# holicc/qurious

Measured on AMD Instinct MI355X. Metric: rows/s on TPC-H Q1 scan+agg and Q3 hash-join, SF10, 1/2/4/8 MI355X, higher is better.
Workload: dtype i128

## Files before the change

### qurious_amd/csrc/agg.cpp

```cpp
#include <hip/hip_runtime_api.h>

#include <algorithm>
#include <cfloat>
#include <cmath>
#include <chrono>
#include <cstdio>
#include <cstdlib>
#include <map>

#include "codegen.hpp"
#include "common.hpp"
#include "device/qhip_status.h"
#include "hostcol.hpp"
#include "jit.hpp"
#include "kargs_host.hpp"
#include "kernels.hpp"
#include "relops.hpp"

namespace qhip {
static uint64_t g_learn_tick = 0;


void HostColumn::init_fixed(const DType& t, int64_t n) {
  type = t; length = n; null_count = 0;
// ... 652 lines not shown
        items_dev.alloc(item_first.size() * 4);
        QHIP_HIP_CHECK(hipMemcpyAsync(items_dev.ptr, item_first.data(), item_first.size() * 4, hipMemcpyHostToDevice, s));
        HReduceLaunch rl;
        rl.records = records.as<uint64_t>();
        rl.item_first = items_dev.as<uint32_t>();
        rl.n_items = n_items;
        HAggLaunch Lp = L;
        Lp.l_nslots = l_nslots_p;
        void* rargs[] = {&rl, &Lp};
        if (wide) {
          std::shared_ptr<Module> m_wide = get_module(ctx, plan.source, "qk_agg_reduce_wide");
          const unsigned rgrid = (unsigned)std::min<uint64_t>(n_items, (uint64_t)ctx->num_cus * 2);
          QHIP_HIP_CHECK(hipModuleLaunchKernel(m_wide->fn, rgrid, 1, 1, 1024, 1, 1, (unsigned)((size_t)l_nslots_p * slot_bytes), s, rargs, nullptr));
        } else {
          const unsigned rgrid = (unsigned)std::min<uint64_t>(n_items, (uint64_t)ctx->num_cus * 4);
          QHIP_HIP_CHECK(hipModuleLaunchKernel(m_red->fn, rgrid, 1, 1, 256, 1, 1, (unsigned)((size_t)l_nslots_p * slot_bytes), s, rargs, nullptr));
        }
        QHIP_HIP_CHECK(sync_stream(s));
      }
      }

    } else if (N > 0 && parts) {
      dense.alloc((size_t)guess * slot_bytes + 8);
      dense_dev = dense.as<uint64_t>();
      L.part_runs = parts->runs; L.part_stride = parts->stride;
      L.dense_out = dense_dev + 1; L.dense_counter = status_dev + 16; L.dense_cap = guess;
      L.n_parts = (uint32_t)parts->n_parts;
      L.part_max = (uint32_t)std::max<int64_t>(1024, env_int("QHIP_AGG_PARTS_MAX_FACTOR", 4) * ((N + parts->n_parts - 1) / parts->n_parts));
      const unsigned pgrid = grid + (unsigned)((uint64_t)N / L.part_max) + 1;
      std::shared_ptr<Module> pmod = get_module(ctx, plan.source, "qk_filter_agg_parts");
      QHIP_HIP_CHECK(hipModuleLaunchKernel(pmod->fn, pgrid, 1, 1, 1024, 1, 1, (unsigned)lds_bytes, ctx->stream, args, nullptr));
    } else if (N > 0) {
      if (wide) {
        std::shared_ptr<Module> wmod = get_module(ctx, plan.source, "qk_filter_agg_wide");
        QHIP_HIP_CHECK(hipModuleLaunchKernel(wmod->fn, grid, 1, 1, 1024, 1, 1, (unsigned)lds_bytes, ctx->stream, args, nullptr));
      } else if (cons) {
        std::shared_ptr<Module> cmod = get_module(ctx, plan.source, "qk_filter_agg_cons");
        QHIP_HIP_CHECK(hipModuleLaunchKernel(cmod->fn, grid, 1, 1, 256, 1, 1, (unsigned)lds_bytes, ctx->stream, args, nullptr));
      } else {
        QHIP_HIP_CHECK(hipModuleLaunchKernel(mod->fn, grid, 1, 1, 256, 1, 1, (unsigned)lds_bytes, ctx->stream, args, nullptr));
      }
    }
    time_mark(ctx, 1);
    uint32_t* const counter_dev = status_dev + 16;
    pre_copied = 0;
    if (plan.W == 0) {
      QHIP_HIP_CHECK(hipMemcpyAsync(status_pinned, status_dev, sizeof(status), hipMemcpyDeviceToHost, ctx->stream));
      QHIP_HIP_CHECK(hipMemcpyAsync(pre_host, table_dev, (size_t)slot_bytes, hipMemcpyDeviceToHost, ctx->stream));
    } else {
      if (use_arena) {
        dense_dev = (uint64_t*)(arena->as<uint8_t>() + zero_bytes) ;
        pre_copied = std::min(PRE, guess);
        const bool direct = env_int("QHIP_AGG_PINNED_SLOTS", 1) != 0;
        launch_compact_slots(table_dev, total_slots, plan.slot_words, dense_dev + 1, counter_dev, guess, ctx->stream, direct ? pre_host + 1 : nullptr, pre_copied);
        QHIP_HIP_CHECK(hipMemcpyAsync(status_pinned, status_dev, 64 + 8, hipMemcpyDeviceToHost, ctx->stream));
        if (!direct) QHIP_HIP_CHECK(hipMemcpyAsync(pre_host + 1, dense_dev + 1, (size_t)pre_copied * slot_bytes, hipMemcpyDeviceToHost, ctx->stream));
      } else {
        if (!parts) { dense.alloc((size_t)guess * slot_bytes + 8); dense_dev = dense.as<uint64_t>(); }
        bool utf8_key = false;
        for (auto& kd : plan.keys) utf8_key = utf8_key || kd.type.id == QHIP_UTF8;
        spec_enqueued = false;
        const bool will_spec = replicas == 1 && plan.last_groups >= dev_threshold && !utf8_key && env_int("QHIP_AGG_NO_SPECULATIVE_FINALIZE", 0) == 0;
        const bool direct = !will_spec && !parts && env_int("QHIP_AGG_PINNED_SLOTS", 1) != 0;
        launch_compact_slots(table_dev, total_slots, plan.slot_words, dense_dev + 1, counter_dev, guess, ctx->stream, direct ? pre_host + 1 : nullptr,
                             std::min(PRE, guess));
        if (will_spec) {
          spec = DevFinal();
          const int ncols = n_groups + n_aggs;
          enqueue_device_finalize(spec, dense_dev + 1, guess, counter_dev, status_dev + 32, status_pinned + 32);
          spec_enqueued = true;
          QHIP_HIP_CHECK(hipMemcpyAsync(status_pinned, status_dev, (size_t)(32 + QS_WORDS + ncols) * 4, hipMemcpyDeviceToHost, ctx->stream));
        } else {
          QHIP_HIP_CHECK(hipMemcpyAsync(status_pinned, status_dev, 64 + 8, hipMemcpyDeviceToHost, ctx->stream));
          pre_copied = std::min(PRE, guess);
          if (!direct) QHIP_HIP_CHECK(hipMemcpyAsync(pre_host + 1, dense_dev + 1, (size_t)pre_copied * slot_bytes, hipMemcpyDeviceToHost, ctx->stream));
        }
      }
    }
    if (use_arena) {
      QHIP_HIP_CHECK(hipEventRecord(ctx->ev[2], ctx->stream));
      QHIP_HIP_CHECK(hipMemsetAsync(arena->ptr, 0, zero_bytes, ctx->stream));
      plan.arena_clean = true;
      mark("launched");
      QHIP_HIP_CHECK(sync_event(ctx->ev[2]));
    } else {
      mark("launched");
      QHIP_HIP_CHECK(sync_stream(ctx->stream));
    }
    memcpy(status, status_pinned, sizeof(status));
    if (env_int("QHIP_AGG_PROF", 0)) {
      const double waves = (double)grid * (block / 64);
      fprintf(stderr, "[qhip agg prof] rows %lld grid %u x %d: loads+eval %.0f  cache %.0f  table updates %.0f  cached keys -> table %.0f  merge %.0f  (x256 cycles per wavefront)\n",
              (long long)N, grid, block, status_pinned[8] / waves, status_pinned[9] / waves, status_pinned[10] / waves, status_pinned[11] / waves, status_pinned[12] / waves);
    }
    mark("synchronised");
    trace_point("aggregate: back from its wait");
    verify_pending_sizes(ctx);
    if (in->rows_dev && in->deferred_count() == 0 && n_groups > 0) return no_batches_out();
    if (ctx->timing) QHIP_HIP_CHECK(hipEventElapsedTime(&main_ms, ctx->ev[0], ctx->ev[1]));
    check_status_words(status);
    if (!status[QS_OVERFLOW]) break;
    if (replicas == 1 && cap >= cap_max) fail(QHIP_HIP_ERROR, "group table overflow at maximum capacity (internal error)");
    cap = replicas > 1 ? std::min<uint32_t>(cap_max, std::max<uint32_t>(cap * 16, 1u << 18)) : (uint32_t)std::min<uint64_t>((uint64_t)cap * 16, cap_max);
    replicas = 1;
    ++retries;
  }

  const uint32_t lds_used = status[QS_LDS_USED];
// ... 257 lines not shown
```

### qurious_amd/csrc/device/qhip_device.hpp

```cpp
#pragma once

typedef unsigned char u8;
typedef unsigned short u16;
typedef unsigned int u32;
typedef unsigned long long u64;
typedef long long i64;
typedef __int128 i128;
typedef unsigned __int128 u128;

#define QH_MAXC 24
#define QH_MAXL 24
#define QH_WAVE 64
#define QH_BLOCK 256

struct KCol {
  const void* v;
  const u8* n;
  const u8* d;
};

struct KArgs {
  KCol c[QH_MAXC];
  u64 lit_lo[QH_MAXL];
  i64 lit_hi[QH_MAXL];
// ... 1437 lines not shown
  qh_mask_load<P>(a, A, first, mine, 0, lane);
  qh_mask_load<P>(a, B, first, mine, 1, lane);
  asm volatile("" ::: "memory");
  __builtin_amdgcn_sched_barrier(0);
#define QH_MASK_TRIP(X3, X1, J)                                    \
  qh_mask_finish<P>(a, X3, mask, wave_count, nwords, lane, err);   \
  qh_mask_load<P>(a, X1, first, mine, (J), lane);                  \
  asm volatile("" ::: "memory");                                   \
  __builtin_amdgcn_sched_barrier(0);
  for (i64 j = 0; j < mine; j += 3) {
    QH_MASK_TRIP(A, C, j + 2)
    QH_MASK_TRIP(B, A, j + 3)
    QH_MASK_TRIP(C, B, j + 4)
  }
#undef QH_MASK_TRIP
  qh_report(status, err);
}

__device__ __forceinline__ u32 qh_region(u64 h, u32 n_regions) { return (u32)(((h >> 32) * (u64)n_regions) >> 32); }
template <int W>
__device__ __forceinline__ u32 qh_join_find(const u64* table, u32 base, u32 mask, const u64* k, u32 s) {
  for (u32 probes = 0; probes <= mask; ++probes) {
    const u32 at = base + (s & mask);
    const u64* slot = table + (size_t)at * (1 + W);
    if (slot[0] < QH_READY) return 0xFFFFFFFFu;
    bool eq = true;
#pragma unroll
    for (int w = 0; w < W; ++w) eq &= slot[1 + w] == k[w];
    if (eq) return at;
    ++s;
  }
  return 0xFFFFFFFFu;
}
struct ProbeLaunch {
  const u64* table;
  const u64* bloom;
  const u32* count;
  const u32* start;
  const u32* rows;
  u32* ent_slot;
  u32* ent_row;
  u32* tile_nent;
  u32* tile_total;
  u32* visited;
  u32* status;
  u32 nslots, bloom_mask;
  u32 n_regions;
  u32 slot_bits, bword_bits, stage_cap;
  u32 tiles_per_wave, lds_words;
  u64 dense_min;
  u32 dense_n, dense_words;
  const u32* dense_rank;
  u32 dense_last;
};

__device__ __forceinline__ u64 qh_filter_mask(u32 x) {
  const u32 lo = (1u << (x & 31u)) | (1u << ((x >> 5) & 31u)), hi = (1u << ((x >> 10) & 31u)) | (1u << ((x >> 15) & 31u));
  return ((u64)hi << 32) | lo;
}
__device__ __forceinline__ u32 qh_filter_word(u64 h, u32 word_mask) { return (u32)(h >> 32) & word_mask; }
__device__ __forceinline__ u32 qh_rfilter_word(u64 h, u32 sb, u32 wb) { return ((u32)h >> sb) & ((1u << wb) - 1u); }
__device__ __forceinline__ u64 qh_rfilter_mask(u64 h, u32 sb, u32 wb) { return qh_filter_mask((u32)(h >> (sb + wb))); }

template <class P>
struct QhProbeTile {
  typename P::Raw raw[P::PROBE_R];
  u64 k[P::PROBE_R][P::W];
  u64 fw[P::PROBE_R], fm[P::PROBE_R];
  u32 at[P::PROBE_R];
  u64 st[P::PROBE_R], kw[P::PROBE_R][P::W];
  bool ok[P::PROBE_R];
  i64 tile;
  bool live;
};
struct QhProbeCtx { bool regions; u32 smask; int lane; i64 first, mine; u32 nent, total; };

template <class P>
__device__ __forceinline__ void qh_probe_stage1(const KArgs& a, QhProbeTile<P>& x, const QhProbeCtx& c, i64 j) {
  constexpr int R = P::PROBE_R, TILE = 64 * R;
  x.live = j < c.mine;
  x.tile = x.live ? c.first + j : 0;
  const i64 tb = x.tile * TILE;
#pragma unroll
  for (int r = 0; r < R; ++r) {
    const u32 o = (u32)r * 64 + (u32)c.lane;
    P::load(a, tb, tb + (i64)o < a.nrows ? o : (u32)(a.nrows - 1 - tb), x.raw[r]);
  }
}
template <class P, bool REGIONS>
__device__ __forceinline__ void qh_probe_stage2(const KArgs& a, const ProbeLaunch& L, QhProbeTile<P>& x, const QhProbeCtx& c, u32& err) {
  constexpr int R = P::PROBE_R, TILE = 64 * R, W = P::W;
#pragma unroll
  for (int r = 0; r < R; ++r) {
    const bool inb = x.tile * TILE + r * 64 + c.lane < a.nrows;
    u32 e = 0;
    x.ok[r] = P::keys(a, x.raw[r], x.k[r], e) && inb;
    err |= (inb && x.live) ? e : 0u;
    const u64 h = qh_key_hash<W>(x.k[r]);
    const u32 reg = REGIONS ? qh_region(h, L.n_regions) : 0u;
    x.at[r] = (REGIONS ? reg << L.slot_bits : 0u) + ((u32)h & c.smask);
    x.fm[r] = REGIONS ? qh_rfilter_mask(h, L.slot_bits, L.bword_bits) : qh_filter_mask((u32)h);
    const u32 word = REGIONS ? (reg << L.bword_bits) + qh_rfilter_word(h, L.slot_bits, L.bword_bits) : qh_filter_word(h, L.bloom_mask);
    x.fw[r] = *(const u64*)((const char*)L.bloom + (size_t)((x.ok[r] ? word : 0u) << 3));
  }
}
template <class P>
// ... 8 lines not shown
      const qh_v2u64 sk = *(const qh_v2u64*)slot;
      x.st[r] = sk.x;
      x.kw[r][0] = sk.y;
    } else {
      x.st[r] = slot[0];
#pragma unroll
      for (int w = 0; w < W; ++w) x.kw[r][w] = slot[1 + w];
    }
  }
}
template <class P>
__device__ __forceinline__ void qh_probe_stage4(const ProbeLaunch& L, QhProbeTile<P>& x, QhProbeCtx& c) {
  constexpr int R = P::PROBE_R, TILE = 64 * R, W = P::W;
  const int lane = c.lane;
  u32 sid[R];
#pragma unroll
  for (int r = 0; r < R; ++r) {
    sid[r] = 0xFFFFFFFFu;
    if (x.ok[r] && x.st[r] >= QH_READY) {
      bool eq = true;
#pragma unroll
      for (int w = 0; w < W; ++w) eq &= x.kw[r][w] == x.k[r][w];
      const u32 home = x.at[r] & c.smask, base = x.at[r] & ~c.smask;
      sid[r] = eq ? x.at[r] : qh_join_find<W>(L.table, base, c.smask, x.k[r], home + 1);
      if (!L.start && sid[r] != 0xFFFFFFFFu) sid[r] = (u32)((eq ? x.st[r] : L.table[(size_t)sid[r] * (1 + W)]) - 2);
    }
  }
  if (!x.live) return;
  u32 total = 0, nent = c.nent;
#pragma unroll
  for (int r = 0; r < R; ++r) {
    const bool found = sid[r] != 0xFFFFFFFFu;
    u32 cnt = 1u;
    if (L.start) cnt = L.count[found ? sid[r] : 0u];
    total += found ? cnt : 0u;
    const u64 m = qh_ballot(found);
    if (found) {
      const size_t pos = (size_t)c.first * TILE + nent + (u32)__builtin_popcountll(m & ((1ULL << lane) - 1));
      L.ent_slot[pos] = sid[r];
      L.ent_row[pos] = (u32)(x.tile * TILE + r * 64 + lane);
    }
    nent += (u32)__builtin_popcountll(m);
  }
  c.nent = nent;
  if (L.visited) {
#pragma unroll
    for (int r = 0; r < R; ++r)
      if (sid[r] != 0xFFFFFFFFu) {
        const u32 s0 = L.start ? L.start[sid[r]] : 0u, cnt = L.start ? L.count[sid[r]] : 1u;
        for (u32 q = 0; q < cnt; ++q) { const u32 b = L.start ? L.rows[s0 + q] : sid[r]; atomicOr(&L.visited[b >> 5], 1u << (b & 31)); }
      }
  }
  c.total += (u32)qh_wave_sum_u64(total);
}

template <class P, bool REGIONS>
__device__ __forceinline__ void qh_join_probe_body(const KArgs& a, const ProbeLaunch& L) {
  constexpr int R = P::PROBE_R, TILE = 64 * R, NW = QH_BLOCK / 64;
  const i64 ntiles = (a.nrows + TILE - 1) / TILE;
  QhProbeCtx c;
  c.regions = REGIONS;
  c.smask = REGIONS ? (1u << L.slot_bits) - 1u : L.nslots - 1u;
  c.lane = qh_lane();
  const i64 wave = (i64)blockIdx.x * NW + __builtin_amdgcn_readfirstlane((int)(threadIdx.x >> 6));
  c.first = wave * (i64)L.tiles_per_wave;
  c.nent = 0; c.total = 0;
  if (c.first >= ntiles) {
    if (c.lane == 0) { L.tile_total[wave] = 0; L.tile_nent[wave] = 0; }
    return;
  }
  c.mine = ntiles - c.first < (i64)L.tiles_per_wave ? ntiles - c.first : (i64)L.tiles_per_wave;
  u32 err = 0;
  QhProbeTile<P> A, B, C;
  qh_probe_stage1<P>(a, A, c, 0);
  qh_probe_stage2<P, REGIONS>(a, L, A, c, err);
  qh_probe_stage1<P>(a, B, c, 1);
  qh_probe_stage3<P>(L, A, c);
  qh_probe_stage2<P, REGIONS>(a, L, B, c, err);
  qh_probe_stage1<P>(a, C, c, 2);
#define QH_PROBE_TRIP(X4, X3, X2, J)          \
  qh_probe_stage4<P>(L, X4, c);               \
  qh_probe_stage3<P>(L, X3, c);               \
  qh_probe_stage2<P, REGIONS>(a, L, X2, c, err);       \
  qh_probe_stage1<P>(a, X4, c, (J));
  for (i64 j = 3; j < c.mine + 3; j += 3) {
    QH_PROBE_TRIP(A, B, C, j)
    QH_PROBE_TRIP(B, C, A, j + 1)
    QH_PROBE_TRIP(C, A, B, j + 2)
  }
#undef QH_PROBE_TRIP
  if (c.lane == 0) { L.tile_total[wave] = c.total; L.tile_nent[wave] = c.nent; }
  qh_report(L.status, err);
}

struct DenseBuildLaunch {
  u32* bits;
  u32* row_of;
  u32* status;
  u64 kmin;
  u32 n;
  u32 gen;
  u8* bytes;
  u32* counters;
};
template <class P, bool DEVROWS = false>
__device__ __forceinline__ void qh_join_dense_build_body(const KArgs& a, const DenseBuildLaunch& L) {
  constexpr int R = 4;
  const i64 nrows = DEVROWS ? qh_rows(a) : a.nrows;
  const i64 tile = (i64)QH_BLOCK * R;
  u32 err = 0, dup = 0, out_of_range = 0, inserted = 0;
  const bool bytemap = L.bytes != nullptr;
  for (i64 tb = (i64)blockIdx.x * tile; tb < nrows; tb += (i64)gridDim.x * tile) {
    u64 k[R][P::W];
    bool ok[R];
#pragma unroll
    for (int r = 0; r < R; ++r) {
      const i64 i = tb + (i64)r * QH_BLOCK + threadIdx.x;
      const bool inb = i < nrows;
      u32 e = 0;
      ok[r] = P::keys(a, inb ? i : nrows - 1, k[r], e) && inb;
      err |= inb ? e : 0u;
    }
#pragma unroll
    for (int r = 0; r < R; ++r) {
      const u64 idx = k[r][0] - L.kmin;
      if (ok[r]) {
        if (idx < (u64)L.n) {
          if (bytemap) {
            L.bytes[(u32)idx] = (u8)L.gen;
            ++inserted;
          } else {
            const u32 bit = 1u << ((u32)idx & 31u);
            const u32 old = __hip_atomic_fetch_or(&L.bits[(u32)idx >> 5], bit, __ATOMIC_RELAXED, __HIP_MEMORY_SCOPE_AGENT);
            dup |= (old & bit) ? 1u : 0u;
          }
          L.row_of[(u32)idx] = (u32)(tb + (i64)r * QH_BLOCK + threadIdx.x);
        } else out_of_range = 1u;
      }
    }
  }
  qh_report(L.status, err | (out_of_range << QS_OVERFLOW));
  if (bytemap) {
    const u32 wave_rows = (u32)qh_wave_sum_u64((u64)inserted);
    if (qh_lane() == 0 && wave_rows) atomicAdd(&L.counters[0], wave_rows);
    return;
// ... 159 lines not shown
  const u64 below = (1ULL << lane) - 1;
  if (st.nbuf + (u32)TILE > st.cap) qh_dense_flush(L, st, (u64)c.first * TILE, lane);
  bool hit[R];
  u64 m[R];
#pragma unroll
  for (int r = 0; r < R; ++r) {
    const u32 word = (LDSBITS == 2 && (x.idx[r] >> 5) < L.lds_words) ? x.bl[r] : x.bw[r];
    hit[r] = x.ok[r] && ((word >> (x.idx[r] & 31u)) & 1u);
    m[r] = qh_ballot(hit[r]);
  }
  if (WIDE) {
    u32 before = 0, total = 0;
#pragma unroll
    for (int r = 0; r < R; ++r) { before += (u32)__builtin_popcountll(m[r] & below); total += (u32)__builtin_popcountll(m[r]); }
    u32 pos = st.nbuf + before;
#pragma unroll
    for (int r = 0; r < R; ++r)
      if (hit[r]) { st.idx[pos] = x.idx[r]; st.row[pos] = (u32)(x.tb + (i64)((u32)lane * R + (u32)r)); ++pos; }
    st.nbuf += total;
  } else {
    u32 n = st.nbuf;
#pragma unroll
    for (int r = 0; r < R; ++r) {
      if (hit[r]) {
        const u32 pos = n + (u32)__builtin_popcountll(m[r] & below);
        st.idx[pos] = x.idx[r];
        st.row[pos] = (u32)(x.tile * TILE + r * 64 + lane);
      }
      n += (u32)__builtin_popcountll(m[r]);
    }
    st.nbuf = n;
  }
}
template <class P, int LDSBITS, bool WIDE>
__device__ __forceinline__ void qh_join_probe_dense_body(const KArgs& a, const ProbeLaunch& L) {
  constexpr int R = P::PROBE_R, TILE = 64 * R;
  const int NW = (int)(blockDim.x >> 6);
  const u32 nbits = LDSBITS == 1 ? L.dense_words : LDSBITS == 2 ? L.lds_words : 0u;
  if (LDSBITS) {
    u32* lbits = (u32*)qh_dyn_lds;
    for (u32 w = threadIdx.x; w < nbits; w += blockDim.x) lbits[w] = ((const u32*)L.bloom)[w];
    __syncthreads();
  }
  const i64 ntiles = (a.nrows + TILE - 1) / TILE;
  QhProbeCtx c;
  c.regions = false; c.smask = 0;
  c.lane = qh_lane();
  const int wave_in_wg = __builtin_amdgcn_readfirstlane((int)(threadIdx.x >> 6));
  const i64 wave = (i64)blockIdx.x * NW + wave_in_wg;
  c.first = wave * (i64)L.tiles_per_wave;
  c.nent = 0; c.total = 0;
  if (c.first >= ntiles) {
    if (c.lane == 0) { L.tile_total[wave] = 0; L.tile_nent[wave] = 0; }
    return;
  }
  c.mine = ntiles - c.first < (i64)L.tiles_per_wave ? ntiles - c.first : (i64)L.tiles_per_wave;
  QhDenseStage st;
  st.cap = L.stage_cap;
  st.idx = (u32*)qh_dyn_lds + ((nbits + 1u) & ~1u) + (u32)wave_in_wg * 2u * L.stage_cap;
  st.row = st.idx + L.stage_cap;
  st.nbuf = 0; st.nflushed = 0;
  u32 err = 0;
  QhDenseTile<P> A, B, C;
  qh_dense_stage1<P, WIDE>(a, A, c, 0);
  qh_dense_stage1<P, WIDE>(a, B, c, 1);
  asm volatile("" ::: "memory");
  qh_dense_stage2<P, LDSBITS, WIDE>(a, L, A, c, err);
  asm volatile("" ::: "memory");
#define QH_DENSE_TRIP(X3, X2, X1, J)                   \
  qh_dense_stage3<P, LDSBITS, WIDE>(L, X3, c, st);     \
  qh_dense_stage2<P, LDSBITS, WIDE>(a, L, X2, c, err); \
  qh_dense_stage1<P, WIDE>(a, X1, c, (J));             \
  asm volatile("" ::: "memory");
  for (i64 j = 0; j < c.mine; j += 3) {
    QH_DENSE_TRIP(A, B, C, j + 2)
    QH_DENSE_TRIP(B, C, A, j + 3)
    QH_DENSE_TRIP(C, A, B, j + 4)
  }
#undef QH_DENSE_TRIP
  qh_dense_flush(L, st, (u64)c.first * TILE, c.lane);
  if (c.lane == 0) { L.tile_total[wave] = st.nflushed; L.tile_nent[wave] = st.nflushed; }
  qh_report(L.status, err);
}

struct ScatterLaunch {
  u64* entries;
  u32* first;
  u32* status;
  u32 n_regions;
  u32 rows_per_wg;
};

#define QH_SCATTER_BLOCK 1024
template <class P, bool DEVROWS = false>
__device__ __forceinline__ void qh_join_scatter_body(const KArgs& a, const ScatterLaunch& L) {
  constexpr int R = 4, W = P::W, TB = QH_SCATTER_BLOCK;
  u32* cnt = (u32*)qh_dyn_lds;
  __shared__ u32 wsum[TB / 64];
  const u32 tid = threadIdx.x, nr = L.n_regions;
  for (u32 r = tid; r <= nr; r += TB) cnt[r] = 0;
  __syncthreads();
  const i64 first = (i64)blockIdx.x * L.rows_per_wg;
  const i64 nrows = DEVROWS ? qh_rows(a) : a.nrows;
  const i64 last = first + L.rows_per_wg < nrows ? first + L.rows_per_wg : nrows;
  u32 err = 0;
  const bool single = last - first <= (i64)TB * R;
  u64 k[R][W];
  bool ok[R];
  for (int pass = 0; pass < 2; ++pass) {
    for (i64 tb = first; tb < last; tb += (i64)TB * R) {
      if (!single || pass == 0) {
#pragma unroll
        for (int r = 0; r < R; ++r) {
          const i64 i = tb + (i64)r * TB + tid;
          const bool inb = i < last;
          u32 e = 0;
          ok[r] = P::keys(a, inb ? i : last - 1, k[r], e) && inb;
          if (pass == 0) err |= inb ? e : 0u;
        }
      }
#pragma unroll
      for (int r = 0; r < R; ++r) {
        if (ok[r]) {
          const u32 reg = qh_region(qh_key_hash<W>(k[r]), nr);
          const u32 pos = atomicAdd(&cnt[reg], 1u);
          if (pass == 1) {
            u64* e = L.entries + ((size_t)first + pos) * (1 + W);
            e[0] = (u64)(tb + (i64)r * TB + tid) + 2;
#pragma unroll
            for (int w = 0; w < W; ++w) e[1 + w] = k[r][w];
          }
        }
      }
    }
    __syncthreads();
// ... 106 lines not shown
```

### qurious_amd/csrc/join.cpp

```cpp
#include <hip/hip_runtime_api.h>

#include <algorithm>
#include <map>

#include "common.hpp"
#include "device/qhip_status.h"
#include "jit.hpp"
#include "kargs_host.hpp"
#include "kernels.hpp"
#include "relops.hpp"

using namespace qhip;

namespace {

uint32_t pow2_ceil32(uint64_t x) {
  uint64_t p = 1;
  while (p < x) p <<= 1;
  return (uint32_t)std::min<uint64_t>(p, 1ULL << 31);
}
int log2u(uint32_t x) { int b = 0; while ((1u << b) < x) ++b; return b; }

uint64_t fnv1a64(const std::string& str, uint64_t h = 1469598103934665603ULL) {
  for (unsigned char c : str) { h ^= c; h *= 1099511628211ULL; }
// ... 315 lines not shown
  DevBuf ent_slot((P + 1) * 4), ent_row((P + 1) * 4), cnt, pair_off, b_idx, p_idx;
  std::string probe_name = dense ? "qk_join_probe_dense" : "qk_join_probe";
  uint64_t M = 0;
  const uint32_t* deferred_slot = nullptr;
  const bool mat_key = dense && unique_keys && join_type == QHIP_JOIN_INNER && froot < 0 && n_on == 1 && rex[on_r[0]].kind == QHIP_EXPR_COLUMN &&
                       rex[on_r[0]].column >= 0 && rex[on_r[0]].column < (int)R->cols.size() && R->cols[(size_t)rex[on_r[0]].column].type.id == QHIP_INT64 &&
                       env_int("QHIP_JOIN_KEY_MATERIALIZE", 1) != 0;
  std::shared_ptr<DevBuf> key_vals;
  std::shared_ptr<DevBuf> rows_blk;
  std::shared_ptr<uint64_t> rows_final;
  bool probe_timed = false;
  const bool want_pairs = !(semi_anti && froot < 0);
  const bool mark_in_probe = has_tail && froot < 0;
  if (P > 0) {
    const uint64_t kProbeTileRows = (uint64_t)64 * (uint64_t)rkp.probe_r;
    const uint32_t stage_extra = (uint32_t)std::max(0, env_int("QHIP_DENSE_STAGE_EXTRA", 256));
    const uint32_t stage_cap_small = (uint32_t)kProbeTileRows + stage_extra, stage_cap_lds = (uint32_t)kProbeTileRows + 128;
    const uint32_t kLdsWords = (160 * 1024 - 16 * 2 * 4 * stage_cap_lds) / 4 - 2;
    const int lds_mode = env_int("QHIP_JOIN_DENSE_LDS", 1);
    const char* probe_kernel = region_build ? "qk_join_probe" : "qk_join_probe_onetable";
    uint32_t lds_words = 0;
    if (dense) {
      probe_kernel = "qk_join_probe_dense";
      if (P >= kProbeTileRows) {
        if (env_int("QHIP_JOIN_DENSE_WIDE", 1) != 0) probe_kernel = "qk_join_probe_dense_wide";
        const bool pays = lds_mode == 2 || (lds_mode == 1 && P >= (1u << 20) && P >= 32ull * std::min(dense_words, kLdsWords) && dense_words <= 2 * kLdsWords);
        if (pays && dense_words <= kLdsWords) { probe_kernel = "qk_join_probe_dense_lds"; lds_words = dense_words; }
        else if (pays) { probe_kernel = "qk_join_probe_dense_hybrid"; lds_words = kLdsWords; }
      }
    }
    const bool dense_lds = lds_words > 0;
    probe_name = probe_kernel;
    std::shared_ptr<Module>& rmod = jp->rmods[probe_kernel];
    if (!rmod) rmod = get_module(ctx, rkp.source, probe_kernel);
    const std::shared_ptr<Module>& mod = rmod;
    HKArgs ka;
    fill_kargs(ctx, R, rkp.bind, ka, jp->rstr);
    const uint64_t ntiles = (P + kProbeTileRows - 1) / kProbeTileRows;
    const unsigned waves_per_wg = dense_lds ? 16 : 4;
    const size_t dyn_lds = !dense ? 0 : (((size_t)lds_words + 1) & ~(size_t)1) * 4 + (size_t)waves_per_wg * 2 * 4 * (dense_lds ? stage_cap_lds : stage_cap_small);
    if (mod->wgs_per_cu == 0 || mod->wgs_dyn_lds != dyn_lds) {
      int nb = 0;
      if (hipModuleOccupancyMaxActiveBlocksPerMultiprocessor(&nb, mod->fn, (int)waves_per_wg * 64, dyn_lds) != hipSuccess || nb < 1) nb = 1;
      mod->wgs_per_cu = nb;
      mod->wgs_dyn_lds = dyn_lds;
    }
    const uint64_t resident = (uint64_t)ctx->num_cus * (uint64_t)mod->wgs_per_cu * waves_per_wg;
    const uint64_t tpw_max = (uint64_t)std::max(1, env_int("QHIP_PROBE_TILES_PER_WAVE", 32));
    const uint64_t rounds = std::max<uint64_t>(1, (ntiles + resident * tpw_max - 1) / (resident * tpw_max));
    const uint64_t waves_wanted = std::min<uint64_t>(ntiles, rounds * resident);
    const uint64_t tiles_per_wave = (ntiles + waves_wanted - 1) / waves_wanted;
    const unsigned grid = (unsigned)std::max<uint64_t>(1, ((ntiles + tiles_per_wave - 1) / tiles_per_wave + waves_per_wg - 1) / waves_per_wg);
    const uint64_t nchunks = (uint64_t)grid * waves_per_wg;
    DevBuf tile_tot((nchunks + 1) * 4), tile_nent((nchunks + 1) * 4);
    HProbeLaunch pl;
    pl.table = table; pl.bloom = bloom; pl.count = count; pl.start = start_ptr; pl.rows = rows_ptr;
    pl.ent_slot = ent_slot.as<uint32_t>();
    pl.ent_row = ent_row.as<uint32_t>();
    pl.tile_nent = tile_nent.as<uint32_t>();
    pl.tile_total = tile_tot.as<uint32_t>();
    pl.visited = (mark_in_probe && !want_pairs) ? visited.as<uint32_t>() : nullptr;
    pl.status = dstat + QS_WORDS;
    pl.nslots = nslots; pl.bloom_mask = filter_words - 1;
    pl.n_regions = n_regions; pl.slot_bits = slot_bits; pl.bword_bits = bword_bits;
    pl.tiles_per_wave = (uint32_t)tiles_per_wave;
    if (dense) {
      pl.count = nullptr;
      pl.stage_cap = dense_lds ? stage_cap_lds : stage_cap_small;
      pl.dense_min = (uint64_t)kmin; pl.dense_n = (uint32_t)dense_n; pl.dense_words = dense_words; pl.lds_words = lds_words;
      pl.dense_rank = dense_rank ? (const uint32_t*)table : nullptr; pl.dense_last = (uint32_t)(B - 1);
    }
    void* args[] = {&ka, &pl};
    time_mark(ctx, 2);
    QHIP_HIP_CHECK(hipModuleLaunchKernel(mod->fn, grid, 1, 1, waves_per_wg * 64, 1, 1, (unsigned)dyn_lds, s, args, nullptr));
    time_mark(ctx, 3);
    probe_timed = true;
    if (want_pairs) exclusive_scan_u32(tile_tot.as<uint32_t>(), tile_tot.as<uint32_t>(), nchunks, dstat + 2 * QS_WORDS, s);
    if (defer) {
      if (!ctx->size_slots) QHIP_HIP_CHECK(hipHostMalloc((void**)&ctx->size_slots, (size_t)kSizeSlots * 32 * 4, hipHostMallocDefault));
      if (ctx->pending_sizes.size() >= (size_t)kSizeSlots) fail(QHIP_HIP_ERROR, "too many joins of deferred size in flight (internal error)");
      uint32_t* slot = ctx->size_slots + (size_t)(ctx->size_slot_next++ % kSizeSlots) * 32;
      auto total_out = std::make_shared<uint64_t>(~0ull);
      ctx->pending_sizes.push_back({slot, size_key, defer_cap, dup_hint, total_out});
      rows_final = total_out;
      M = defer_cap;
      b_idx.alloc((M + 1) * 4);
      p_idx.alloc((M + 1) * 4);
      rows_blk = std::make_shared<DevBuf>(64);
      if (mat_key) key_vals = std::make_shared<DevBuf>((M + 1) * 8);
      launch_join_emit(ent_slot.as<uint32_t>(), ent_row.as<uint32_t>(), tile_nent.as<uint32_t>(), tile_tot.as<uint32_t>(), count, start_ptr, rows_ptr, dense && !dense_rank ? (const uint32_t*)table : nullptr, nchunks, tiles_per_wave * kProbeTileRows, b_idx.as<uint32_t>(), p_idx.as<uint32_t>(),
                       nullptr, nullptr, nullptr, (uint32_t)M, dstat, slot, rows_blk->as<uint32_t>(), s, key_vals ? key_vals->as<int64_t>() : nullptr, (uint64_t)kmin,
                       dense_rank ? (const uint32_t*)table : nullptr, (const uint32_t*)bloom, dense ? (uint32_t)(B - 1) : 0xFFFFFFFFu);
      deferred_slot = slot;
    } else {
    QHIP_HIP_CHECK(hipMemcpyAsync(st_build, dstat, (2 * QS_WORDS + 1) * 4, hipMemcpyDeviceToHost, s));
    QHIP_HIP_CHECK(sync_stream(s));
    verify_pending_sizes(ctx);
    if (speculate) {
      if (order_broken()) return hash_join(ctx, L, R, join_type, lex, nlex, rex, nrex, on_l, on_r, n_on, fex, nfex, froot, fsides, fcols, nfcols, lpred, rpred);
      check_build_status();
      if (max_count > 1) {
        if (ctx->join_dup_builds.size() > 4096) ctx->join_dup_builds.clear();
        ctx->join_dup_builds.insert(dup_hint);
        return hash_join(ctx, L, R, join_type, lex, nlex, rex, nrex, on_l, on_r, n_on, fex, nfex, froot, fsides, fcols, nfcols, lpred, rpred);
      }
    }
    check_status_words(st);
    M = st[QS_WORDS];
    if (join_type == QHIP_JOIN_INNER && froot < 0) {
      if (ctx->join_size_hints.size() > 4096) ctx->join_size_hints.clear();
      ctx->join_size_hints[size_key] = M;
    }
    if (want_pairs) {
      b_idx.alloc((M + 1) * 4);
      p_idx.alloc((M + 1) * 4);
      if (pad_right) {
        cnt.alloc((P + 1) * 4);
        pair_off.alloc((P + 1) * 4);
        QHIP_HIP_CHECK(hipMemsetAsync(cnt.ptr, 0, cnt.bytes, s));
      }
      if (mat_key) key_vals = std::make_shared<DevBuf>((M + 1) * 8);
      launch_join_emit(ent_slot.as<uint32_t>(), ent_row.as<uint32_t>(), tile_nent.as<uint32_t>(), tile_tot.as<uint32_t>(), count, start_ptr, rows_ptr, dense && !dense_rank ? (const uint32_t*)table : nullptr, nchunks, tiles_per_wave * kProbeTileRows, b_idx.as<uint32_t>(), p_idx.as<uint32_t>(),
                       pad_right ? pair_off.as<uint32_t>() : nullptr, pad_right ? cnt.as<uint32_t>() : nullptr,
                       mark_in_probe ? visited.as<uint32_t>() : nullptr, 0xFFFFFFFFu, nullptr, nullptr, nullptr, s, key_vals ? key_vals->as<int64_t>() : nullptr, (uint64_t)kmin,
                       dense_rank ? (const uint32_t*)table : nullptr, (const uint32_t*)bloom, dense ? (uint32_t)(B - 1) : 0xFFFFFFFFu);
    }
    }
    visited_done = mark_in_probe;
  } else if (speculate) {
    QHIP_HIP_CHECK(hipMemcpyAsync(st_build, dstat, QS_WORDS * 4, hipMemcpyDeviceToHost, s));
// ... 203 lines not shown
```

### qurious_amd/csrc/kargs_host.hpp

```cpp
#pragma once
#include <cstdint>

namespace qhip {

constexpr int kMaxCols = 24;
constexpr int kMaxLits = 24;

struct HKCol {
  const void* v;
  const uint8_t* n;
  const uint8_t* d;
};
struct HKArgs {
  HKCol c[kMaxCols];
  uint64_t lit_lo[kMaxLits];
  int64_t lit_hi[kMaxLits];
  const uint8_t* strlit;
  int stroff[kMaxLits + 1];
  int64_t nrows;
  const uint32_t* nrows_dev;
};
static_assert(sizeof(HKCol) == 24, "KCol layout");
static_assert(sizeof(HKArgs) == 24 * 24 + 8 * 24 + 8 * 24 + 8 + 104 + 8 + 8, "KArgs layout");

// ... 16 lines not shown
  uint32_t* hist;
  uint64_t* records;
  uint32_t* status;
  uint32_t n_bins;
  uint32_t rows_per_wg;
};
static_assert(sizeof(HPartLaunch) == 32, "PartLaunch layout");
struct HReduceLaunch {
  const uint64_t* records;
  const uint32_t* item_first;
  uint32_t n_items;
  uint32_t slices = 1;
  const uint32_t* hist = nullptr;
  uint32_t g1 = 0, n_bins = 0, min_slice = 0, pad_ = 0;
};
static_assert(sizeof(HReduceLaunch) == 48, "ReduceLaunch layout");

struct HRunsLaunch {
  uint64_t* dense_out;
  uint32_t* counter;
  uint32_t* status;
  uint32_t* flags;
  uint32_t cap, max_run;
  uint32_t lds_bytes = 0, pad_ = 0;
};
static_assert(sizeof(HRunsLaunch) == 48, "RunsLaunch layout");

struct HProjOut {
  void* v[kMaxCols];
  uint64_t* n[kMaxCols];
  uint8_t* d[kMaxCols];
};
static_assert(sizeof(HProjOut) == 3 * 8 * 24, "ProjOut layout");

struct HProbeLaunch {
  const uint64_t* table;
  const uint64_t* bloom;
  const uint32_t* count;
  const uint32_t* start;
  const uint32_t* rows;
  uint32_t* ent_slot;
  uint32_t* ent_row;
  uint32_t* tile_nent;
  uint32_t* tile_total;
  uint32_t* visited;
  uint32_t* status;
  uint32_t nslots, bloom_mask;
  uint32_t n_regions = 0, slot_bits = 0, bword_bits = 0, stage_cap = 0;
  uint32_t tiles_per_wave = 1, lds_words = 0;
  uint64_t dense_min = 0;
  uint32_t dense_n = 0, dense_words = 0;
  const uint32_t* dense_rank = nullptr;
  uint32_t dense_last = 0, pad_ = 0;
};
static_assert(sizeof(HProbeLaunch) == 11 * 8 + 8 + 16 + 8 + 16 + 16, "ProbeLaunch layout");

struct HDenseBuildLaunch {
  uint32_t* bits;
  uint32_t* row_of;
  uint32_t* status;
  uint64_t kmin;
  uint32_t n;
  uint32_t gen = 0;
  uint8_t* bytes = nullptr;
  uint32_t* counters = nullptr;
};
static_assert(sizeof(HDenseBuildLaunch) == 56, "DenseBuildLaunch layout");

struct HDenseSortedLaunch {
  uint32_t* bits;
  uint32_t* rank = nullptr;
  uint32_t* row_of = nullptr;
  uint32_t* status;
  uint64_t kmin;
  uint32_t n;
  uint32_t words;
};
static_assert(sizeof(HDenseSortedLaunch) == 48, "DenseSortedLaunch layout");
constexpr uint64_t kSortedBuildRows = 1024;
constexpr uint64_t kSortedMaxWords = 16384;

struct HPartIdsLaunch {
  uint8_t* ids;
  uint32_t* hist;
  uint32_t* status;
  uint32_t n_units;
  uint32_t rows_per_unit;
  uint32_t wg_units;
  uint32_t pad_;
  const int64_t* bounds = nullptr;
};
static_assert(sizeof(HPartIdsLaunch) == 48, "PartIdsLaunch layout");

constexpr int kPartMaxCols = 8;
struct HPartScatterLaunch {
  const uint8_t* ids;
  const uint32_t* runs;
  int64_t nrows;
  const uint32_t* nrows_dev;
  uint32_t n_units, rows_per_unit, n_parts, sub;
  void* trash;
  const void* src[kPartMaxCols];
  const uint32_t* idx[kPartMaxCols];
  void* out[kPartMaxCols];
};
static_assert(sizeof(HPartScatterLaunch) == 32 + 16 + 8 + 3 * 8 * 8, "PartScatterLaunch layout");

struct HScatterLaunch {
// ... 10 lines not shown
```

### qurious_amd/csrc/kernels.hip

```cpp
#include <hip/hip_runtime.h>

#include <algorithm>

#include "device/qhip_status.h"
#include "device/qhip_device.hpp"
#include "kernels.hpp"

namespace qhip {

__global__ __launch_bounds__(QH_BLOCK) void k_compact_slots(const u64* table, u32 nslots, int slot_words, u64* out, u32* counter,
                                                            u32 out_capacity, u64* out_host, u32 cap_host) {
  const int lane = qh_lane();
  const u32 nwaves = gridDim.x * (QH_BLOCK / 64), wave = blockIdx.x * (QH_BLOCK / 64) + (threadIdx.x >> 6);
  const u32 per_wave = ((nslots + nwaves - 1) / nwaves + 63) / 64 * 64;
  const u64 lo = (u64)wave * per_wave, hi = lo + per_wave < (u64)nslots ? lo + per_wave : (u64)nslots;
  __shared__ u32 wtot[QH_BLOCK / 64];
  __shared__ u32 wg_base;
  const u32 w = threadIdx.x >> 6;
  u32 mine = 0;
  if (lo < hi) for (u64 s = lo + lane; s < hi; s += 64) mine += table[(size_t)s * slot_words] == QH_READY ? 1u : 0u;
  const u32 total = (u32)qh_wave_sum_u64(mine);
  if (lane == 0) wtot[w] = total;
  __syncthreads();
  if (threadIdx.x == 0) {
    u32 all = 0;
    for (int k = 0; k < QH_BLOCK / 64; ++k) all += wtot[k];
    wg_base = all ? atomicAdd(counter, all) : 0u;
  }
  __syncthreads();
  if (lo >= hi || !total) return;
  u32 base = wg_base;
  for (u32 k = 0; k < w; ++k) base += wtot[k];
  for (u64 s0 = lo; s0 < hi; s0 += 64) {
    const u64 s = s0 + lane;
    const u64* slot = table + (size_t)s * slot_words;
    const bool ready = s < hi && slot[0] == QH_READY;
    const u64 m = qh_ballot(ready);
    if (ready) {
      const u32 idx = base + (u32)__popcll(m & ((1ULL << lane) - 1));
      if (idx < out_capacity) {
        u64* o = out + (size_t)idx * slot_words;
        for (int k = 0; k < slot_words; ++k) o[k] = slot[k];
      }
      if (idx < cap_host) {
        u64* o = out_host + (size_t)idx * slot_words;
        for (int k = 0; k < slot_words; ++k) o[k] = slot[k];
      }
    }
    base += (u32)__popcll(m);
  }
}

static inline unsigned grid_for(uint64_t n, unsigned cap = 2048) {
  uint64_t g = (n + QH_BLOCK - 1) / QH_BLOCK;
  if (g < 1) g = 1;
  if (g > cap) g = cap;
  return (unsigned)g;
}

void launch_compact_slots(const uint64_t* table, uint32_t nslots, int slot_words, uint64_t* out, uint32_t* counter,
                          uint32_t out_capacity, hipStream_t s, uint64_t* out_host, uint32_t cap_host) {
  const unsigned blocks = (unsigned)std::max<uint64_t>(16, std::min<uint64_t>(512, ((uint64_t)nslots + 1023) / 1024));
  hipLaunchKernelGGL(k_compact_slots, dim3(blocks), dim3(QH_BLOCK), 0, s, (const u64*)table, nslots, slot_words, (u64*)out, counter,
                     out_capacity, (u64*)out_host, out_host ? cap_host : 0u);
}

}
```

### qurious_amd/csrc/kernels.hpp

```cpp
#pragma once
#include <hip/hip_runtime_api.h>
#include <cstdint>

namespace qhip {

constexpr uint32_t kNullIdx = 0xFFFFFFFFu;

void launch_compact_slots(const uint64_t* table, uint32_t nslots, int slot_words, uint64_t* out, uint32_t* counter,
                          uint32_t out_capacity, hipStream_t s, uint64_t* out_host = nullptr, uint32_t cap_host = 0);

void exclusive_scan_u32(const uint32_t* in, uint32_t* out, uint64_t n, uint32_t* total_dev, hipStream_t s);
void launch_select_indices(const uint64_t* mask, const uint32_t* wave_offset, uint64_t nrows, uint32_t* sel, hipStream_t s);
void launch_mask_prefix_at(const uint64_t* mask, const uint32_t* wave_offset, const uint64_t* rows, uint32_t n, uint64_t nrows, uint32_t total,
                           uint32_t* out, hipStream_t s);
void launch_mask_from_bits(const uint32_t* bits, uint64_t nrows, int want_set, uint64_t* mask, uint32_t* wave_count, hipStream_t s);
void launch_gather_fixed(const void* in, const uint32_t* idx, void* out, uint64_t m, int width, hipStream_t s);
void launch_compact_fixed(const void* in, const uint64_t* mask, const uint32_t* wave_offset, void* out, uint64_t nrows, int width, hipStream_t s);
void launch_gather_bits(const uint8_t* bitmap, const uint32_t* idx, uint64_t m, uint64_t* out_words, uint32_t* set_count, hipStream_t s);
void launch_gather_utf8_lengths(const int32_t* offsets, const uint32_t* idx, uint64_t m, uint32_t* out_len, hipStream_t s);
void launch_gather_utf8_bytes(const int32_t* offsets, const uint8_t* data, const uint32_t* idx, uint64_t m, const uint32_t* out_off,
                              uint8_t* out_data, hipStream_t s);
void launch_value_maxabs(const void* values, uint64_t n, int words, uint64_t* out, hipStream_t s, uint32_t* narrow32 = nullptr);
void launch_narrow_decimal(const void* values, uint64_t n, int bytes, void* out, hipStream_t s, int src_words = 2);
void launch_pack_field(const void* values, uint64_t n, int width, void* records, uint32_t stride, uint32_t offset, hipStream_t s);
void launch_value_range(const void* values, uint64_t n, int width, bool is_signed, uint64_t* out, hipStream_t s);
void launch_store_u32(uint32_t* p, uint32_t v, hipStream_t s);
void launch_utf8_max_len(const int32_t* offsets, uint64_t n, uint32_t* out, hipStream_t s);
void launch_iota_u32(uint32_t* out, uint64_t n, hipStream_t s, uint32_t first = 0);
void launch_iota_stride_u32(uint32_t* out, uint64_t n, uint32_t stride, hipStream_t s);
void launch_fill_u32(uint32_t* out, uint64_t n, uint32_t v, hipStream_t s);
void launch_lookup_u32(const uint32_t* off, const uint64_t* rows, uint32_t n, uint64_t nrows, uint32_t total, uint32_t* out, hipStream_t s);

void launch_join_build_insert(int W, const uint64_t* keys, const uint64_t* keyvalid, uint64_t n, uint64_t* table, uint32_t nslots,
                              uint32_t* row_slot, uint32_t* extra, uint64_t* bloom, uint32_t bloom_mask, uint32_t* status, hipStream_t s);
void launch_join_region_build(int W, const uint64_t* entries, const uint32_t* first, uint32_t n_wgs, uint32_t rows_per_wg, uint64_t* table,
                              uint64_t* bloom, uint32_t n_regions, uint32_t slot_bits, uint32_t bword_bits, uint32_t* status, hipStream_t s);
void launch_join_full_counts(int W, const uint64_t* table, uint32_t nslots, uint32_t* count, hipStream_t s);
void launch_add_i32(int32_t* p, uint64_t n, int32_t delta, hipStream_t s);
void launch_add_i32_batched(int32_t* p, uint64_t n, const uint64_t* starts, const int32_t* shifts, uint32_t nb, hipStream_t s);
void launch_bits_append(uint32_t* dst, uint64_t dst_pos, const uint8_t* src, uint64_t nbits, hipStream_t s);
void launch_pair_indices(uint32_t* minor, uint32_t* major, uint64_t n, uint32_t n_minor, uint32_t minor0, uint32_t major0, int unused, hipStream_t s);
void launch_count_bits(const uint64_t* words, uint64_t nbits, uint32_t* out, hipStream_t s);
void launch_sort_gather_img(const uint64_t* img, const uint32_t* idx, uint64_t n, uint64_t flip, uint64_t* out, hipStream_t s);
void launch_sort_gather_valid(const uint64_t* validwords, const uint32_t* idx, uint64_t n, bool nulls_first, uint64_t* out, hipStream_t s);
void launch_sort_utf8_chunk(const int32_t* offsets, const uint8_t* data, const uint8_t* validity, const uint32_t* idx, uint64_t n, int chunk,
                            uint64_t flip, uint64_t* out, hipStream_t s);
void stable_sort_pairs_u64(const uint64_t* keys_in, uint64_t* keys_out, const uint32_t* vals_in, uint32_t* vals_out, uint64_t n, int bits,
                           hipStream_t s);
struct GatherDesc { const void* in; const uint32_t* idx; void* out; uint64_t m; uint32_t width; uint32_t null_ones; };
constexpr int kGatherBatch = 8;
struct GatherBatch { GatherDesc d[kGatherBatch]; };
void launch_gather_multi(const GatherBatch& b, int n, hipStream_t s);
void launch_gather_u32_nullable(const uint32_t* inner, const uint32_t* idx, uint32_t* out, uint64_t m, hipStream_t s);
void launch_lower_bound_u32(const uint32_t* a, uint64_t m, const uint32_t* m_dev, const uint64_t* bound, uint32_t nb, uint32_t* pos, hipStream_t s);
void launch_bytes_to_bits(const uint8_t* bytes, uint32_t gen, uint32_t* bits, uint32_t nwords, uint32_t* counters, uint32_t* status, hipStream_t s);
void launch_join_emit(const uint32_t* ent_slot, const uint32_t* ent_row, const uint32_t* chunk_nent, const uint32_t* chunk_off, const uint32_t* count,
                      const uint32_t* start, const uint32_t* rows, const uint32_t* row_of, uint64_t nchunks, uint64_t chunk_rows, uint32_t* b_idx, uint32_t* p_idx,
                      uint32_t* pair_off, uint32_t* cnt_out, uint32_t* visited, uint32_t cap, const uint32_t* stat_block, uint32_t* publish,
                      uint32_t* rows_out, hipStream_t s, int64_t* key_out = nullptr, uint64_t key_min = 0, const uint32_t* rank = nullptr,
                      const uint32_t* rank_bits = nullptr, uint32_t build_last = 0xFFFFFFFFu);
void launch_join_mark(const uint32_t* b_idx, const uint32_t* p_idx, uint64_t m, uint32_t* visited_bits, uint32_t* cnt_per_probe, hipStream_t s);
void launch_join_out_counts(const uint32_t* cnt, uint64_t np, uint32_t* out_cnt, hipStream_t s);
// ... 52 lines not shown
```

Measured before the change: 190.2 billion.

## Fuse probe-offset scan and status publish into last-finishing workgroup

The join probe kernels now end with a last-block-done ticket, and the final workgroup runs an exclusive scan over per-wave tile totals in place. This replaces the separate exclusive_scan_u32 launch when the chunk count is small. Separately, the arena path of the aggregation compaction kernel has its last block publish the status block and counter straight into pinned host memory, replacing a device-to-host memcpy. Both aim to remove kernel/copy launches on the stream. The cost is extra atomics and fences in every block, plus serial tail work done by one workgroup.

Result: slower. 155.8 billion (-18.1%).

```diff
diff --git a/qurious_amd/csrc/agg.cpp b/qurious_amd/csrc/agg.cpp
--- a/qurious_amd/csrc/agg.cpp
+++ b/qurious_amd/csrc/agg.cpp
@@ -728,8 +728,8 @@
         dense_dev = (uint64_t*)(arena->as<uint8_t>() + zero_bytes) ;
         pre_copied = std::min(PRE, guess);
         const bool direct = env_int("QHIP_AGG_PINNED_SLOTS", 1) != 0;
-        launch_compact_slots(table_dev, total_slots, plan.slot_words, dense_dev + 1, counter_dev, guess, ctx->stream, direct ? pre_host + 1 : nullptr, pre_copied);
-        QHIP_HIP_CHECK(hipMemcpyAsync(status_pinned, status_dev, 64 + 8, hipMemcpyDeviceToHost, ctx->stream));
+        launch_compact_slots(table_dev, total_slots, plan.slot_words, dense_dev + 1, counter_dev, guess, ctx->stream, direct ? pre_host + 1 : nullptr, pre_copied,
+                             status_dev, status_pinned);
         if (!direct) QHIP_HIP_CHECK(hipMemcpyAsync(pre_host + 1, dense_dev + 1, (size_t)pre_copied * slot_bytes, hipMemcpyDeviceToHost, ctx->stream));
       } else {
         if (!parts) { dense.alloc((size_t)guess * slot_bytes + 8); dense_dev = dense.as<uint64_t>(); }
diff --git a/qurious_amd/csrc/device/qhip_device.hpp b/qurious_amd/csrc/device/qhip_device.hpp
--- a/qurious_amd/csrc/device/qhip_device.hpp
+++ b/qurious_amd/csrc/device/qhip_device.hpp
@@ -1513,6 +1513,9 @@
   u32 dense_n, dense_words;
   const u32* dense_rank;
   u32 dense_last;
+  u32 pad_;
+  u32* scan_total;
+  u32* scan_ticket;
 };
 
 __device__ __forceinline__ u64 qh_filter_mask(u32 x) {
@@ -1627,6 +1630,56 @@
       }
   }
   c.total += (u32)qh_wave_sum_u64(total);
+}
+
+template <int MAXV>
+__device__ __forceinline__ void qh_scan_u32_one_wg(u32* v, u32 n, u32* total, u32* lds) {
+  typedef u32 qh_v4u __attribute__((ext_vector_type(4)));
+  u32* wsum = lds;
+  const u32 lane = threadIdx.x & 63u, w = threadIdx.x >> 6, nw = blockDim.x >> 6;
+  const u32 per_pass = blockDim.x * (u32)MAXV * 4u;
+  u32 carry = 0;
+  for (u32 base = 0; base < n; base += per_pass) {
+    const u32 first = base + threadIdx.x * (u32)MAXV * 4u;
+    qh_v4u x[MAXV];
+#pragma unroll
+    for (int k = 0; k < MAXV; ++k) {
+      const u32 i = first + (u32)k * 4u;
+      x[k] = (qh_v4u)(0u);
+      if (i < n) x[k] = ((const qh_v4u*)(v + (size_t)first))[k];
+      x[k].y = i + 1u < n ? x[k].y : 0u; x[k].z = i + 2u < n ? x[k].z : 0u; x[k].w = i + 3u < n ? x[k].w : 0u;
+    }
+    u32 sum = 0;
+#pragma unroll
+    for (int k = 0; k < MAXV; ++k) sum += x[k].x + x[k].y + x[k].z + x[k].w;
+    const u32 incl = qh_wave_incl_scan_u32(sum, (int)lane);
+    if (lane == 63u) wsum[w] = incl;
+    __syncthreads();
+    u32 run = carry + incl - sum, all = 0;
+    for (u32 q = 0; q < nw; ++q) { const u32 t = wsum[q]; run += q < w ? t : 0u; all += t; }
+#pragma unroll
+    for (int k = 0; k < MAXV; ++k) {
+      const u32 i = first + (u32)k * 4u;
+      qh_v4u o;
+      o.x = run; o.y = o.x + x[k].x; o.z = o.y + x[k].y; o.w = o.z + x[k].z;
+      if (i < n) ((qh_v4u*)(v + (size_t)first))[k] = o;
+      run = o.w + x[k].w;
+    }
+    carry += all;
+    __syncthreads();
+  }
+  if (threadIdx.x == 0 && total) *total = carry;
+}
+
+__device__ __forceinline__ void qh_probe_scan_epilogue(const ProbeLaunch& L, u32* lds) {
+  if (!L.scan_ticket) return;
+  __threadfence();
+  __syncthreads();
+  if (threadIdx.x == 0) lds[17] = atomicAdd(L.scan_ticket, 1u) == gridDim.x - 1 ? 1u : 0u;
+  __syncthreads();
+  if (!lds[17]) return;
+  __threadfence();
+  qh_scan_u32_one_wg<4>(L.tile_total, gridDim.x * (blockDim.x >> 6), L.scan_total, lds);
 }
 
 template <class P, bool REGIONS>
@@ -1642,8 +1695,7 @@
   c.nent = 0; c.total = 0;
   if (c.first >= ntiles) {
     if (c.lane == 0) { L.tile_total[wave] = 0; L.tile_nent[wave] = 0; }
-    return;
-  }
+  } else {
   c.mine = ntiles - c.first < (i64)L.tiles_per_wave ? ntiles - c.first : (i64)L.tiles_per_wave;
   u32 err = 0;
   QhProbeTile<P> A, B, C;
@@ -1666,6 +1718,9 @@
 #undef QH_PROBE_TRIP
   if (c.lane == 0) { L.tile_total[wave] = c.total; L.tile_nent[wave] = c.nent; }
   qh_report(L.status, err);
+  }
+  __shared__ u32 scan_lds[18];
+  qh_probe_scan_epilogue(L, scan_lds);
 }
 
 struct DenseBuildLaunch {
@@ -1931,8 +1986,7 @@
   c.nent = 0; c.total = 0;
   if (c.first >= ntiles) {
     if (c.lane == 0) { L.tile_total[wave] = 0; L.tile_nent[wave] = 0; }
-    return;
-  }
+  } else {
   c.mine = ntiles - c.first < (i64)L.tiles_per_wave ? ntiles - c.first : (i64)L.tiles_per_wave;
   QhDenseStage st;
   st.cap = L.stage_cap;
@@ -1960,6 +2014,8 @@
   qh_dense_flush(L, st, (u64)c.first * TILE, c.lane);
   if (c.lane == 0) { L.tile_total[wave] = st.nflushed; L.tile_nent[wave] = st.nflushed; }
   qh_report(L.status, err);
+  }
+  qh_probe_scan_epilogue(L, (u32*)qh_dyn_lds);
 }
 
 struct ScatterLaunch {
diff --git a/qurious_amd/csrc/join.cpp b/qurious_amd/csrc/join.cpp
--- a/qurious_amd/csrc/join.cpp
+++ b/qurious_amd/csrc/join.cpp
@@ -391,7 +391,7 @@
     const uint64_t tiles_per_wave = (ntiles + waves_wanted - 1) / waves_wanted;
     const unsigned grid = (unsigned)std::max<uint64_t>(1, ((ntiles + tiles_per_wave - 1) / tiles_per_wave + waves_per_wg - 1) / waves_per_wg);
     const uint64_t nchunks = (uint64_t)grid * waves_per_wg;
-    DevBuf tile_tot((nchunks + 1) * 4), tile_nent((nchunks + 1) * 4);
+    DevBuf tile_tot((nchunks + 4) * 4), tile_nent((nchunks + 1) * 4);
     HProbeLaunch pl;
     pl.table = table; pl.bloom = bloom; pl.count = count; pl.start = start_ptr; pl.rows = rows_ptr;
     pl.ent_slot = ent_slot.as<uint32_t>();
@@ -409,12 +409,15 @@
       pl.dense_min = (uint64_t)kmin; pl.dense_n = (uint32_t)dense_n; pl.dense_words = dense_words; pl.lds_words = lds_words;
       pl.dense_rank = dense_rank ? (const uint32_t*)table : nullptr; pl.dense_last = (uint32_t)(B - 1);
     }
+    const int scan_mode = env_int("QHIP_PROBE_SCAN_EPILOGUE", 1);
+    const bool scan_in_probe = want_pairs && (scan_mode == 2 || (scan_mode == 1 && nchunks <= (uint64_t)waves_per_wg * 64 * 16));
+    if (scan_in_probe) { pl.scan_total = dstat + 2 * QS_WORDS; pl.scan_ticket = dstat + 2 * QS_WORDS + 1; }
     void* args[] = {&ka, &pl};
     time_mark(ctx, 2);
     QHIP_HIP_CHECK(hipModuleLaunchKernel(mod->fn, grid, 1, 1, waves_per_wg * 64, 1, 1, (unsigned)dyn_lds, s, args, nullptr));
     time_mark(ctx, 3);
     probe_timed = true;
-    if (want_pairs) exclusive_scan_u32(tile_tot.as<uint32_t>(), tile_tot.as<uint32_t>(), nchunks, dstat + 2 * QS_WORDS, s);
+    if (want_pairs && !scan_in_probe) exclusive_scan_u32(tile_tot.as<uint32_t>(), tile_tot.as<uint32_t>(), nchunks, dstat + 2 * QS_WORDS, s);
     if (defer) {
       if (!ctx->size_slots) QHIP_HIP_CHECK(hipHostMalloc((void**)&ctx->size_slots, (size_t)kSizeSlots * 32 * 4, hipHostMallocDefault));
       if (ctx->pending_sizes.size() >= (size_t)kSizeSlots) fail(QHIP_HIP_ERROR, "too many joins of deferred size in flight (internal error)");
diff --git a/qurious_amd/csrc/kargs_host.hpp b/qurious_amd/csrc/kargs_host.hpp
--- a/qurious_amd/csrc/kargs_host.hpp
+++ b/qurious_amd/csrc/kargs_host.hpp
@@ -92,8 +92,10 @@
   uint32_t dense_n = 0, dense_words = 0;
   const uint32_t* dense_rank = nullptr;
   uint32_t dense_last = 0, pad_ = 0;
+  uint32_t* scan_total = nullptr;
+  uint32_t* scan_ticket = nullptr;
 };
-static_assert(sizeof(HProbeLaunch) == 11 * 8 + 8 + 16 + 8 + 16 + 16, "ProbeLaunch layout");
+static_assert(sizeof(HProbeLaunch) == 11 * 8 + 8 + 16 + 8 + 16 + 16 + 16, "ProbeLaunch layout");
 
 struct HDenseBuildLaunch {
   uint32_t* bits;
diff --git a/qurious_amd/csrc/kernels.hip b/qurious_amd/csrc/kernels.hip
--- a/qurious_amd/csrc/kernels.hip
+++ b/qurious_amd/csrc/kernels.hip
@@ -9,13 +9,13 @@
 namespace qhip {
 
 __global__ __launch_bounds__(QH_BLOCK) void k_compact_slots(const u64* table, u32 nslots, int slot_words, u64* out, u32* counter,
-                                                            u32 out_capacity, u64* out_host, u32 cap_host) {
+                                                            u32 out_capacity, u64* out_host, u32 cap_host, u32* stat_block, u32* publish) {
   const int lane = qh_lane();
   const u32 nwaves = gridDim.x * (QH_BLOCK / 64), wave = blockIdx.x * (QH_BLOCK / 64) + (threadIdx.x >> 6);
   const u32 per_wave = ((nslots + nwaves - 1) / nwaves + 63) / 64 * 64;
   const u64 lo = (u64)wave * per_wave, hi = lo + per_wave < (u64)nslots ? lo + per_wave : (u64)nslots;
   __shared__ u32 wtot[QH_BLOCK / 64];
-  __shared__ u32 wg_base;
+  __shared__ u32 wg_base, wg_last;
   const u32 w = threadIdx.x >> 6;
   u32 mine = 0;
   if (lo < hi) for (u64 s = lo + lane; s < hi; s += 64) mine += table[(size_t)s * slot_words] == QH_READY ? 1u : 0u;
@@ -26,8 +26,19 @@
     u32 all = 0;
     for (int k = 0; k < QH_BLOCK / 64; ++k) all += wtot[k];
     wg_base = all ? atomicAdd(counter, all) : 0u;
+    u32 last = 0;
+    if (publish) {
+      __threadfence();
+      last = atomicAdd(&stat_block[18], 1u) == gridDim.x - 1 ? 1u : 0u;
+    }
+    wg_last = last;
   }
   __syncthreads();
+  if (wg_last && threadIdx.x < 18) {
+    __threadfence();
+    publish[threadIdx.x] = threadIdx.x == 16 ? __hip_atomic_load(counter, __ATOMIC_RELAXED, __HIP_MEMORY_SCOPE_AGENT) : threadIdx.x == 17 ? 0u : stat_block[threadIdx.x];
+    __threadfence_system();
+  }
   if (lo >= hi || !total) return;
   u32 base = wg_base;
   for (u32 k = 0; k < w; ++k) base += wtot[k];
@@ -59,10 +70,10 @@
 }
 
 void launch_compact_slots(const uint64_t* table, uint32_t nslots, int slot_words, uint64_t* out, uint32_t* counter,
-                          uint32_t out_capacity, hipStream_t s, uint64_t* out_host, uint32_t cap_host) {
+                          uint32_t out_capacity, hipStream_t s, uint64_t* out_host, uint32_t cap_host, uint32_t* stat_block, uint32_t* publish) {
   const unsigned blocks = (unsigned)std::max<uint64_t>(16, std::min<uint64_t>(512, ((uint64_t)nslots + 1023) / 1024));
   hipLaunchKernelGGL(k_compact_slots, dim3(blocks), dim3(QH_BLOCK), 0, s, (const u64*)table, nslots, slot_words, (u64*)out, counter,
-                     out_capacity, (u64*)out_host, out_host ? cap_host : 0u);
+                     out_capacity, (u64*)out_host, out_host ? cap_host : 0u, (u32*)stat_block, (u32*)(stat_block ? publish : nullptr));
 }
 
 }
diff --git a/qurious_amd/csrc/kernels.hpp b/qurious_amd/csrc/kernels.hpp
--- a/qurious_amd/csrc/kernels.hpp
+++ b/qurious_amd/csrc/kernels.hpp
@@ -7,7 +7,8 @@
 constexpr uint32_t kNullIdx = 0xFFFFFFFFu;
 
 void launch_compact_slots(const uint64_t* table, uint32_t nslots, int slot_words, uint64_t* out, uint32_t* counter,
-                          uint32_t out_capacity, hipStream_t s, uint64_t* out_host = nullptr, uint32_t cap_host = 0);
+                          uint32_t out_capacity, hipStream_t s, uint64_t* out_host = nullptr, uint32_t cap_host = 0,
+                          uint32_t* stat_block = nullptr, uint32_t* publish = nullptr);
 
 void exclusive_scan_u32(const uint32_t* in, uint32_t* out, uint64_t n, uint32_t* total_dev, hipStream_t s);
 void launch_select_indices(const uint64_t* mask, const uint32_t* wave_offset, uint64_t nrows, uint32_t* sel, hipStream_t s);
```
